# CliqueOfficial/zk-dcap-verifier

Measured on AMD Instinct MI355X. Metric: proofs/hour sgx_dcap_verifier k=19 (create_proof on the GPU: commitments, lookups, grand products, NTTs, evaluate_h, evaluations, SHPLONK, host transcript; witness synthesis excluded), higher is better.
Workload: dtype u32x8 (256-bit Montgomery integers)

## Files before the change

### zk-dcap-verifier_amd/csrc/capi.hip

```cpp
#include <string.h>
#include <new>
#include <system_error>
#include "quotient.h"

namespace zk {
int ntt_set_lds_attr();
int quotient_set_lds_attr();
int domain_lagrange_to_coeff(zk_ctx* ctx, void* d_a, uint32_t k);
int domain_coeff_to_lagrange(zk_ctx* ctx, void* d_a, uint32_t k);
int domain_lagrange_to_coeff_batch(zk_ctx* ctx, void* const* cols, size_t count, uint32_t k);
int domain_coeff_to_extended_batch(zk_ctx* ctx, const void* const* coeffs, void* const* outs, size_t count, uint32_t k, uint32_t ek);
int ntt_dev_batch(zk_ctx* ctx, void* const* h_cols, const void* const* h_srcs, size_t count, uint32_t log_n, const u256& omega, const NttFuse* fuse);
int domain_coeff_to_extended(zk_ctx* ctx, const void* d_coeff, uint32_t k, uint32_t ek, void* d_out);
int domain_extended_to_coeff(zk_ctx* ctx, void* d_a, uint32_t k, uint32_t ek);
int domain_divide_by_vanishing(zk_ctx* ctx, void* d_a, uint32_t k, uint32_t ek);
int fr_vec_op(zk_ctx* ctx, int op, const void* a, const void* b, void* out, size_t n, const u256* scalar);
int permutation_product(zk_ctx* ctx, const void* const* values, const void* const* sigmas, size_t count, uint32_t k, const void* beta, const void* gamma,
                        const void* delta_start, const void* z_init, const void* blinding, uint32_t bf, void* d_z, void* h_last_z);
int lookup_product(zk_ctx* ctx, const void* cin, const void* ctab, const void* pin, const void* ptab, uint32_t k, const void* beta, const void* gamma,
                   const void* blinding, uint32_t bf, void* d_z);
int permutation_product_circuits(zk_ctx* ctx, const void* const* values, const void* const* sigmas, size_t m, size_t n_circuits, uint32_t chunk_len, uint32_t k,
                                 const void* beta, const void* gamma, const void* blinding, uint32_t bf, void* const* d_zs);
int lookup_product_batch(zk_ctx* ctx, const void* const* cols4, size_t count, uint32_t k, const void* beta, const void* gamma, const void* blinding,
                         uint32_t bf, void* const* d_zs);
// ... 181 lines not shown
        t = ctx->tune; timing = ctx->timing;
    }
    std::lock_guard<std::mutex> lk(h->mu);
    h->tune = t;
    h->timing = timing;
    return h;
}
static void release_workspaces(zk_ctx* ctx) {
    zk::DevBuf* bufs[] = {&ctx->ws_scalars, &ctx->ws_sorted, &ctx->ws_mid, &ctx->ws_small, &ctx->ws_sub0, &ctx->ws_sub1, &ctx->ws_cls0,
                          &ctx->ws_cls1, &ctx->ws_tmp, &ctx->ws_ntt, &ctx->ws_ntt_in, &ctx->ws_pts, &ctx->ws_runs, &ctx->ws_quot, &ctx->ws_quot_state};
    for (auto* b : bufs) b->release();
}
void zk_internal_trim_helper(zk_ctx* ctx) {
    if (!ctx) return;
    zk_ctx* h;
    { LOCK; h = ctx->helper; }
    if (!h) return;
    std::lock_guard<std::mutex> lk(h->mu);
    (void)hipSetDevice(h->device);
    (void)hipStreamSynchronize(h->stream);
    release_workspaces(h);
    release_twiddles(h);
}
extern "C" {
void zk_ctx_destroy(zk_ctx* ctx) ZK_ABI_TRY {
    if (!ctx) return;
    zk_ctx* helper;
    { LOCK; helper = ctx->helper; ctx->helper = nullptr; }
    if (helper) zk_ctx_destroy(helper);
    zk_internal_plonk_ctx_destroyed(ctx);
    (void)zk_plonk_trim(ctx);
    {
        LOCK;
        (void)hipSetDevice(ctx->device);
        (void)hipStreamSynchronize(ctx->stream);
        ctx->bases.clear();
        drop_pending_timers(ctx);
        release_twiddles(ctx);
        release_pks(ctx);
        release_mock_sessions(ctx);
        release_programs(ctx);
        release_gtab(ctx);
        release_workspaces(ctx);
        (void)hipStreamDestroy(ctx->stream);
    }
    delete ctx;
} ZK_ABI_CATCH_VOID(ctx)

const char* zk_last_error(zk_ctx* ctx) ZK_ABI_TRY { return ctx ? ctx->err : "null context"; } ZK_ABI_CATCH_VALUE(ctx, "zkmi355: internal error")

static int* tune_slot(zk_ctx* ctx, const char* key) {
    zk::Tune& t = ctx->tune;
    struct { const char* k; int* v; } tab[] = {
        {"msm_c", &t.msm_c}, {"msm_sort_wgs", &t.msm_sort_wgs}, {"msm_sort_threads", &t.msm_sort_threads}, {"msm_sort_batch_wgs", &t.msm_sort_batch_wgs}, {"msm_bsort_threads", &t.msm_bsort_threads}, {"msm_bsort_chunk", &t.msm_bsort_chunk}, {"msm_wide_bins_log", &t.msm_wide_bins_log}, {"msm_part_threads", &t.msm_part_threads}, {"msm_part_pairs", &t.msm_part_pairs}, {"msm_two_level_sort", &t.msm_two_level_sort},
        {"msm_target_threads", &t.msm_target_threads}, {"msm_min_chunk", &t.msm_min_chunk}, {"msm_max_chunk", &t.msm_max_chunk},
        {"msm_max_chunk_wide", &t.msm_max_chunk_wide}, {"msm_merge_fanin", &t.msm_merge_fanin}, {"msm_tree_fanin", &t.msm_tree_fanin}, {"msm_block", &t.msm_block}, {"msm_runs", &t.msm_runs}, {"prover_side_lane", &t.prover_side_lane}, {"prover_lane_priority", &t.prover_lane_priority},
        {"ntt_tile_log", &t.ntt_tile_log}, {"ntt_threads", &t.ntt_threads}, {"ntt_max_radix_log", &t.ntt_max_radix_log}, {"ntt_plan", &t.ntt_plan}, {"ntt_full_twiddle_max_log", &t.ntt_full_twiddle_max_log}, {"ntt_coset_table", &t.ntt_coset_table}, {"ntt_col_major", &t.ntt_col_major},
        {"vec_block", &t.vec_block}, {"quot_threads", &t.quot_threads},
        {"ntt_quarter_input", &t.ntt_quarter_input}, {"ntt_fuse_scale", &t.ntt_fuse_scale}, {"quot_piece_cosets", &t.quot_piece_cosets}, {"quot_factor_horner", &t.quot_factor_horner}, {"quot_degree_split", &t.quot_degree_split}, {"quot_group_factors", &t.quot_group_factors}, {"ntt_ws_limit_mb", &t.ntt_ws_limit_mb}, 
        {"quot_jit", &t.quot_jit}, {"quot_jit_group", &t.quot_jit_group}, {"quot_jit_waves", &t.quot_jit_waves}, {"quot_remat_ops", &t.quot_remat_ops}, {"quot_remat_distance", &t.quot_remat_distance}, {"keygen_wgs", &t.keygen_wgs}, {"mock_edge_wgs", &t.mock_edge_wgs}};
    for (auto& e : tab) if (!strcmp(e.k, key)) return e.v;
    return nullptr;
}
int zk_tune_set(zk_ctx* ctx, const char* key, int value) ZK_ABI_TRY {
    NEED_CTX; LOCK;
    int* s = key ? tune_slot(ctx, key) : nullptr;
    if (!s) return ctx->fail(ZK_ERR_ARG, "zk_tune_set: unknown key '%s'", key ? key : "(null)");
    if (value < 0) return ctx->fail(ZK_ERR_ARG, "zk_tune_set: negative value");
    *s = value;
    return ZK_OK;
} ZK_ABI_CATCH(ctx)
int zk_tune_get(zk_ctx* ctx, const char* key, int* value) ZK_ABI_TRY {
    NEED_CTX; LOCK;
    int* s = key ? tune_slot(ctx, key) : nullptr;
    if (!s || !value) return ctx->fail(ZK_ERR_ARG, "zk_tune_get: unknown key '%s'", key ? key : "(null)");
    *value = *s;
    return ZK_OK;
} ZK_ABI_CATCH(ctx)
int zk_timing_enable(zk_ctx* ctx, int on) ZK_ABI_TRY {
    NEED_CTX;
    zk_ctx* helper;
    { LOCK; helper = ctx->helper; }
    if (helper) (void)zk_timing_enable(helper, on);
    LOCK;
    resolve_pending_timers(ctx);
    if (on) ctx->last_ms.clear();
    ctx->timing = on != 0;
    return ZK_OK;
} ZK_ABI_CATCH(ctx)
double zk_timing_get(zk_ctx* ctx, const char* label) ZK_ABI_TRY {
    if (!ctx || !label) return -1.0;
    zk_ctx* helper;
    { LOCK; helper = ctx->helper; }
    const double side = helper ? zk_timing_get(helper, label) : -1.0;
    LOCK;
    resolve_pending_timers(ctx);
    auto it = ctx->last_ms.find(label);
    if (it == ctx->last_ms.end()) return side;
    return it->second + (side > 0 ? side : 0.0);
} ZK_ABI_CATCH_VALUE(ctx, -1.0)

#define ENTER NEED_CTX; LOCK; ZK_HIP(hipSetDevice(ctx->device))

int zk_dev_alloc(zk_ctx* ctx, size_t bytes, void** dptr) ZK_ABI_TRY { ENTER; if (!dptr) return ctx->fail(ZK_ERR_ARG, "null"); ZK_HIP(hipMalloc(dptr, bytes ? bytes : 32)); return ZK_OK; } ZK_ABI_CATCH(ctx)
int zk_dev_free(zk_ctx* ctx, void* dptr) ZK_ABI_TRY { ENTER; ZK_HIP(hipFree(dptr)); return ZK_OK; } ZK_ABI_CATCH(ctx)
int zk_dev_upload(zk_ctx* ctx, void* dptr, const void* host, size_t bytes) ZK_ABI_TRY {
    ENTER; if ((!dptr || !host) && bytes) return ctx->fail(ZK_ERR_ARG, "zk_dev_upload: null");
// ... 285 lines not shown
```

### zk-dcap-verifier_amd/csrc/ctx.h

```cpp
#pragma once
#include <stdarg.h>
#include <string.h>
#include <stdio.h>
#include <list>
#include <map>
#include <memory>
#include <mutex>
#include <string>
#include <vector>
#include "ec.cuh"
#include "../../include/zkmi355.h"
#include "abi_guard.h"

namespace zk {

struct Tune {
    int msm_c = 0;
    int msm_sort_wgs = 256;
    int msm_sort_threads = 1024;
    int msm_bsort_threads = 1024;
    int msm_bsort_chunk = 8192;
    int msm_part_threads = 1024, msm_part_pairs = 16384;
    int msm_wide_bins_log = 9;
    int msm_two_level_sort = 0;
    int msm_sort_batch_wgs = 2048;
    int msm_target_threads = 1 << 19;
    int msm_min_chunk = 16;
    int msm_max_chunk = 48;
    int msm_max_chunk_wide = 128;
    int msm_merge_fanin = 8;
    int msm_tree_fanin = 2;
    int msm_block = 128;
    int prover_lane_priority = 1;
    int prover_side_lane = 1;
    int msm_runs = 1;
    int ntt_tile_log = 10;
    int ntt_threads = 256;
    int ntt_max_radix_log = 8;
    int ntt_plan = 0;
    int ntt_col_major = 1;
    int ntt_coset_table = 1;
    int ntt_full_twiddle_max_log = 24;
    int ntt_ws_limit_mb = 24576;
    int ntt_fuse_scale = 1;
    int ntt_quarter_input = 1;
    int vec_block = 256;
    int quot_threads = 128;
    int quot_piece_cosets = 1;
    int quot_degree_split = 1;
    int quot_group_factors = 1;
    int quot_factor_horner = 1;
    int quot_remat_ops = 4;
    int quot_remat_distance = 24;
    int quot_jit = 0;
    int quot_jit_waves = 0;
    int keygen_wgs = 2048;
    int mock_edge_wgs = 2048;
    int quot_jit_group = 200;
};

struct DevBuf {
    void* p = nullptr;
    size_t cap = 0;
    hipError_t ensure(size_t bytes) {
        if (bytes <= cap) return hipSuccess;
        if (p) (void)hipFree(p);
        p = nullptr; cap = 0;
        size_t want = bytes + bytes / 8 + 4096;
        hipError_t e = hipMalloc(&p, want);
        if (e == hipSuccess) cap = want;
        return e;
    }
    void release() { if (p) (void)hipFree(p); p = nullptr; cap = 0; }
};

struct DevTmp {
    void* p = nullptr;
    DevTmp() = default;
// ... 81 lines not shown
#define ZK_CHECK_LAUNCH() ZK_HIP(hipGetLastError())

namespace zk {
inline void resolve_pending_timers(zk_ctx* ctx);
struct EvTimer {
    zk_ctx* ctx; const char* label; hipEvent_t a = nullptr, b = nullptr; bool on;
    EvTimer(zk_ctx* c, const char* l) : ctx(c), label(l), on(c->timing) {
        if (on) { (void)hipEventCreate(&a); (void)hipEventCreate(&b); (void)hipEventRecord(a, ctx->stream); }
    }
    void stop() { if (on) (void)hipEventRecord(b, ctx->stream); }
    void resolve() {
        if (!on) return;
        (void)hipEventSynchronize(b);
        float ms = 0; (void)hipEventElapsedTime(&ms, a, b);
        on = false;
        (void)hipEventDestroy(a); (void)hipEventDestroy(b);
        ctx->last_ms[label] += ms; ctx->last_ms[std::string(label) + "#n"] += 1.0;
    }
    void defer() {
        if (!on) return;
        if (ctx->pending_timers.size() >= 4096) resolve_pending_timers(ctx);
        ctx->pending_timers.push_back({label, a, b});
        on = false;
    }
    ~EvTimer() { if (on) { (void)hipEventDestroy(a); (void)hipEventDestroy(b); } }
    EvTimer(const EvTimer&) = delete;
    EvTimer& operator=(const EvTimer&) = delete;
};
inline void resolve_pending_timers(zk_ctx* ctx) {
    std::vector<zk_ctx::PendingTimer> list;
    list.swap(ctx->pending_timers);
    struct Drop { std::vector<zk_ctx::PendingTimer>& l; ~Drop() { for (auto& t : l) { (void)hipEventDestroy(t.a); (void)hipEventDestroy(t.b); } } } drop{list};
    for (auto& t : list) {
        (void)hipEventSynchronize(t.b);
        float ms = 0; (void)hipEventElapsedTime(&ms, t.a, t.b);
        ctx->last_ms[t.label] += ms; ctx->last_ms[std::string(t.label) + "#n"] += 1.0;
    }
}
inline void drop_pending_timers(zk_ctx* ctx) {
    for (auto& t : ctx->pending_timers) { (void)hipEventDestroy(t.a); (void)hipEventDestroy(t.b); }
    ctx->pending_timers.clear();
}

int msm_register(zk_ctx* ctx, const void* pts, size_t n, bool on_device, uint64_t* handle);
int msm_release(zk_ctx* ctx, uint64_t handle);
int msm_share(zk_ctx* dst, const BaseTable& bt, uint64_t* handle);
int msm_enable_runs(zk_ctx* ctx, uint64_t handle);
int msm_run(zk_ctx* ctx, uint64_t handle, const void* scalars, size_t n, bool on_device, void* out, int partial);
int msm_run_batch(zk_ctx* ctx, uint64_t handle, const void* const* scalars, size_t nb, size_t n, bool on_device, void* out, int partial);
int g1_sum_xyzz_host(const void* xyzz, size_t count, void* out_jac);
int g1_fixed_base_mul(zk_ctx* ctx, const void* d_scalars, size_t n, void* d_out_affine);
void release_gtab(zk_ctx* ctx);
int msm_set_lds_attr();
struct NttFuse {
    const void* src = nullptr;
    uint32_t n_valid = 0;
    int pre_zeta = 0;
    int post_scale = 0;
    u256 scale;
    int post_zeta_inv = 0;
    const void* cs_lo = nullptr; const void* cs_hi = nullptr; uint32_t cs_lo_bits = 0, cs_stride = 0, cs_log = 0;
    const void* pre_full = nullptr;
};
int ntt_dev(zk_ctx* ctx, void* d_a, uint32_t log_n, const u256& omega, const NttFuse* fuse);
void release_twiddles(zk_ctx* ctx);
void release_programs(zk_ctx* ctx);
void release_mock_sessions(zk_ctx* ctx);
int quotient_program_share(zk_ctx* ctx, zk_ctx* owner, uint64_t owner_prog, uint64_t* prog);
}
```

### zk-dcap-verifier_amd/csrc/msm.hip

```cpp
#include "ctx.h"
#include <algorithm>
#include <math.h>

namespace zk {

template <class F>
ZK_HD void for_each_digit(u256 s, int c, int W, F&& f) {
    const uint32_t mask = (1u << c) - 1u, half = 1u << (c - 1);
    uint32_t carry = 0;
    for (int j = 0; j < W; j++) {
        uint32_t d = (s.v[0] & mask) + carry;
#pragma unroll
        for (int i = 0; i < 7; i++) s.v[i] = (s.v[i] >> c) | (s.v[i + 1] << (32 - c));
        s.v[7] >>= c;
        if (d > half) {
            carry = 1;
            uint32_t m = (1u << c) - d;
            if (m) f(j, m, true);
        } else {
            carry = 0;
            if (d) f(j, d, false);
        }
    }
}
// ... 28 lines not shown
        if (d > 0x8000u) {
            carry = 1;
            const uint32_t m = 0x10000u - d;
            if (m) f(j, m, true);
        } else {
            carry = 0;
            if (d) f(j, d, false);
        }
    }
}
template <int J = 0, class F>
ZK_HD void for_each_digit16_static(const u256& s, F&& f, uint32_t carry = 0) {
    if constexpr (J < 16) {
        const uint32_t d = ((s.v[J >> 1] >> (16 * (J & 1))) & 0xffffu) + carry;
        uint32_t cy = 0;
        if (d > 0x8000u) {
            cy = 1;
            const uint32_t m = 0x10000u - d;
            if (m) f(WinIdx<J>{}, m, true);
        } else if (d) f(WinIdx<J>{}, d, false);
        for_each_digit16_static<J + 1>(s, f, cy);
    }
}

ZK_HD uint32_t find_segment(const uint32_t* arr, uint32_t B, uint32_t j) {
    uint32_t lo = 0, hi = B;
    while (hi - lo > 1) {
        uint32_t mid = (lo + hi) >> 1;
        if (arr[mid] <= j) lo = mid; else hi = mid;
    }
    return lo;
}

ZK_HD uint32_t ceil_div(uint32_t a, uint32_t b) { return (a + b - 1) / b; }

constexpr int MSM_MAX_LEVELS = 12;
struct MsmPlan {
    uint32_t n, n_table, B, L, M, Mlog, R, nb;
    int c, W;
    const void* const* scalars;
    const void* table;
    const void* const* col_tables;
    uint32_t* small;
    uint32_t small_stride, o_off, o_cursor, o_suboff, o_info, o_tiles, o_fulloff, o_remorder, o_remhist, o_remstart, o_remcursor;
    uint32_t* sorted;
    uint64_t sorted_stride;
    uint32_t low_bits, nbin, pch, bch, o_bintot, o_bincur, o_binbase, o_chunkbase;
    uint32_t* mid_ref;
    uint16_t* mid_low;
    void* sub[2];
    uint64_t sub_stride[2];
    void* cls[2];
    uint32_t lo_bits;
};
ZK_HD uint32_t* plan_small(const MsmPlan& p, uint32_t col) { return p.small + (size_t)col * p.small_stride; }
ZK_HD const uint32_t* plan_suboff(const MsmPlan& p, uint32_t col, uint32_t level) { return plan_small(p, col) + p.o_suboff + (size_t)level * (p.B + 1); }
ZK_HD uint32_t plan_eff_levels(const MsmPlan& p, uint32_t max_s) {
    uint32_t pw = 1, r = 0;
    while (pw < max_s && r < p.R) { pw *= p.M; r++; }
    return r;
}

constexpr uint32_t MSM_MAX_BINS = 2048, MSM_MAX_LOW = 8192;
constexpr int MSM_MAX_C = 22;

__device__ __forceinline__ void block_incscan(uint32_t* v, uint32_t* tmp, uint32_t N) {
    for (uint32_t d = 1; d < N; d <<= 1) {
        for (uint32_t t = threadIdx.x; t < N; t += blockDim.x) tmp[t] = v[t] + (t >= d ? v[t - d] : 0u);
        __syncthreads();
        for (uint32_t t = threadIdx.x; t < N; t += blockDim.x) v[t] = tmp[t];
        __syncthreads();
    }
}

ZK_KERNEL void msm_bin_hist_kernel(MsmPlan p) {
    __shared__ uint32_t lh[MSM_MAX_BINS];
    const uint32_t col = blockIdx.y;
    const void* scalars = p.scalars[col];
    for (uint32_t b = threadIdx.x; b < p.nbin; b += blockDim.x) lh[b] = 0;
    __syncthreads();
    const uint32_t chunk = ceil_div(p.n, gridDim.x);
    const uint32_t lo = blockIdx.x * chunk;
    const uint32_t hi = lo + chunk < p.n ? lo + chunk : p.n;
    for (uint32_t i = lo + threadIdx.x; i < hi; i += blockDim.x) {
        u256 s = Fr::from_mont(load_u256(scalars, i));
        for_each_digit(s, p.c, p.W, [&](int, uint32_t mag, bool) { atomicAdd(&lh[(mag - 1) >> p.low_bits], 1u); });
    }
    __syncthreads();
    uint32_t* tot = plan_small(p, col) + p.o_bintot;
    for (uint32_t b = threadIdx.x; b < p.nbin; b += blockDim.x) {
        uint32_t v = lh[b];
        if (v) atomicAdd(&tot[b], v);
    }
}

ZK_KERNEL void msm_bin_base_kernel(MsmPlan p) {
    __shared__ uint32_t v[MSM_MAX_BINS], w[MSM_MAX_BINS], tmp[MSM_MAX_BINS];
    uint32_t* sm = plan_small(p, blockIdx.x);
    for (uint32_t b = threadIdx.x; b < p.nbin; b += blockDim.x) { const uint32_t t = sm[p.o_bintot + b]; v[b] = t; w[b] = ceil_div(t, p.bch); }
    __syncthreads();
    block_incscan(v, tmp, p.nbin);
    block_incscan(w, tmp, p.nbin);
    for (uint32_t b = threadIdx.x; b < p.nbin; b += blockDim.x) { sm[p.o_binbase + b + 1] = v[b]; sm[p.o_chunkbase + b + 1] = w[b]; }
    if (threadIdx.x == 0) { sm[p.o_binbase] = 0; sm[p.o_chunkbase] = 0; }
}

// ... 85 lines not shown
#pragma unroll
        for (uint32_t u = 0; u < BS_U; u++) { const uint32_t e = e0 + u * blockDim.x; k[u] = e < hi ? mlow[e] : 0xffffffffu; }
#pragma unroll
        for (uint32_t u = 0; u < BS_U; u++) if (k[u] != 0xffffffffu) atomicAdd(&cnt[k[u]], 1u);
    }
    __syncthreads();
    uint32_t* hist = sm + (size_t)bin * nlow;
    for (uint32_t b = threadIdx.x; b < nlow; b += blockDim.x) {
        const uint32_t v = cnt[b];
        if (v) atomicAdd(&hist[b], v);
    }
}
ZK_KERNEL void msm_bsort_place_kernel(MsmPlan p) {
    ZK_DYN_SHARED(uint32_t, cnt);
    const uint32_t col = blockIdx.y, nlow = 1u << p.low_bits;
    uint32_t* sm = plan_small(p, col);
    uint32_t bin, lo, hi;
    if (!bsort_chunk(p, sm, bin, lo, hi)) return;
    for (uint32_t b = threadIdx.x; b < nlow; b += blockDim.x) cnt[b] = 0;
    __syncthreads();
    const uint32_t* __restrict__ mref = p.mid_ref + (size_t)col * p.sorted_stride;
    const uint16_t* __restrict__ mlow = p.mid_low + (size_t)col * p.sorted_stride;
    for (uint32_t e0 = lo + threadIdx.x; e0 < hi; e0 += BS_U * blockDim.x) {
        uint32_t k[BS_U];
#pragma unroll
        for (uint32_t u = 0; u < BS_U; u++) { const uint32_t e = e0 + u * blockDim.x; k[u] = e < hi ? mlow[e] : 0xffffffffu; }
#pragma unroll
        for (uint32_t u = 0; u < BS_U; u++) if (k[u] != 0xffffffffu) atomicAdd(&cnt[k[u]], 1u);
    }
    __syncthreads();
    uint32_t* cursor = sm + p.o_cursor + (size_t)bin * nlow;
    for (uint32_t b0 = threadIdx.x; b0 < nlow; b0 += 4 * blockDim.x) {
        uint32_t v[4], r[4];
#pragma unroll
        for (int u = 0; u < 4; u++) { const uint32_t b = b0 + u * blockDim.x; v[u] = b < nlow ? cnt[b] : 0u; }
#pragma unroll
        for (int u = 0; u < 4; u++) r[u] = v[u] ? atomicAdd(&cursor[b0 + u * blockDim.x], v[u]) : 0u;
#pragma unroll
        for (int u = 0; u < 4; u++) { const uint32_t b = b0 + u * blockDim.x; if (b < nlow) cnt[b] = r[u]; }
    }
    __syncthreads();
    uint32_t* __restrict__ sorted = p.sorted + (size_t)col * p.sorted_stride;
    for (uint32_t e0 = lo + threadIdx.x; e0 < hi; e0 += BS_U * blockDim.x) {
        uint32_t k[BS_U], r[BS_U], d[BS_U];
#pragma unroll
        for (uint32_t u = 0; u < BS_U; u++) { const uint32_t e = e0 + u * blockDim.x; const bool in = e < hi; k[u] = in ? mlow[e] : 0xffffffffu; r[u] = in ? mref[e] : 0u; }
#pragma unroll
        for (uint32_t u = 0; u < BS_U; u++) d[u] = k[u] != 0xffffffffu ? atomicAdd(&cnt[k[u]], 1u) : 0u;
#pragma unroll
        for (uint32_t u = 0; u < BS_U; u++) if (k[u] != 0xffffffffu) sorted[d[u]] = r[u];
    }
}

ZK_KERNEL void msm_hist_kernel(MsmPlan p) {
    ZK_DYN_SHARED(uint32_t, lh);
    const uint32_t B = p.B, col = blockIdx.y;
    const void* scalars = p.scalars[col];
    for (uint32_t b = threadIdx.x; b < B; b += blockDim.x) lh[b] = 0;
    __syncthreads();
    const uint32_t chunk = ceil_div(p.n, gridDim.x);
    const uint32_t lo = blockIdx.x * chunk;
    const uint32_t hi = lo + chunk < p.n ? lo + chunk : p.n;
    const bool wide16 = p.c == 16 && p.W == 16;
    for (uint32_t i = lo + threadIdx.x; i < hi; i += blockDim.x) {
        u256 s = Fr::from_mont(load_u256(scalars, i));
        if (wide16) for_each_digit16(s, [&](int, uint32_t mag, bool) { atomicAdd(&lh[mag - 1], 1u); });
        else for_each_digit(s, p.c, p.W, [&](int, uint32_t mag, bool) { atomicAdd(&lh[mag - 1], 1u); });
    }
    __syncthreads();
    uint32_t* ghist = plan_small(p, col);
    for (uint32_t b = threadIdx.x; b < B; b += blockDim.x) {
        uint32_t v = lh[b];
        if (v) atomicAdd(&ghist[b], v);
    }
}


constexpr uint32_t SC_SPT = 4, SC_WMAX = 32;
ZK_KERNEL void msm_scatter_kernel(MsmPlan p) {
    ZK_DYN_SHARED(uint32_t, lh);
    const uint32_t B = p.B, col = blockIdx.y;
    const void* scalars = p.scalars[col];
    for (uint32_t b = threadIdx.x; b < B; b += blockDim.x) lh[b] = 0;
    const bool wide16 = p.c == 16 && p.W == 16;
    const uint32_t chunk = ceil_div(p.n, gridDim.x);
    const uint32_t lo = blockIdx.x * chunk;
    const uint32_t hi = lo + chunk < p.n ? lo + chunk : p.n;
    u256 sc[SC_SPT];
    uint32_t rk[SC_SPT][SC_WMAX / 2] = {};
#pragma unroll
    for (uint32_t u = 0; u < SC_SPT; u++) {
        const uint32_t i = lo + threadIdx.x + u * blockDim.x;
        if (i < hi) sc[u] = load_u256(scalars, i);
    }
    __syncthreads();
#pragma unroll
    for (uint32_t u = 0; u < SC_SPT; u++) {
        const uint32_t i = lo + threadIdx.x + u * blockDim.x;
        if (i < hi) {
            sc[u] = Fr::from_mont(sc[u]);
            auto count = [&](auto jc, uint32_t mag, bool) {
                constexpr int j = decltype(jc)::value;
                const uint32_t r = atomicAdd(&lh[mag - 1], 1u);
                if (j & 1) rk[u][j / 2] |= r << 16; else rk[u][j / 2] = r;
            };
            if (wide16) for_each_digit16_static(sc[u], count);
            else { u256 t = sc[u]; for_each_digit_static<SC_WMAX>(t, p.c, p.W, count); }
        }
    }
    __syncthreads();
    uint32_t* cursor = plan_small(p, col) + p.o_cursor;
    for (uint32_t b0 = threadIdx.x; b0 < B; b0 += 8 * blockDim.x) {
        uint32_t v[8], r[8];
#pragma unroll
        for (int u = 0; u < 8; u++) { const uint32_t b = b0 + u * blockDim.x; v[u] = b < B ? lh[b] : 0u; }
#pragma unroll
        for (int u = 0; u < 8; u++) r[u] = v[u] ? atomicAdd(&cursor[b0 + u * blockDim.x], v[u]) : 0u;
#pragma unroll
        for (int u = 0; u < 8; u++) { const uint32_t b = b0 + u * blockDim.x; if (b < B) lh[b] = r[u]; }
    }
    __syncthreads();
    uint32_t* sorted = p.sorted + (size_t)col * p.sorted_stride;
#pragma unroll
    for (uint32_t u = 0; u < SC_SPT; u++) {
        const uint32_t i = lo + threadIdx.x + u * blockDim.x;
        if (i < hi) {
            auto place = [&](auto jc, uint32_t mag, bool neg) {
                constexpr int j = decltype(jc)::value;
                const uint32_t r = (j & 1) ? rk[u][j / 2] >> 16 : rk[u][j / 2] & 0xffffu;
                sorted[lh[mag - 1] + r] = (neg ? 0x80000000u : 0u) | ((uint32_t)j * p.n_table + i);
            };
            if (wide16) for_each_digit16_static(sc[u], place);
            else for_each_digit_static<SC_WMAX>(sc[u], p.c, p.W, place);
        }
    }
}

constexpr uint32_t SC_T = 256, SC_E = 4, SC_TILE = SC_T * SC_E, SC_NV = MSM_MAX_LEVELS + 3, REM_CLASSES = 256;
struct ScanVals { uint32_t v[SC_NV]; };
ZK_HD uint32_t rem_class(uint32_t r) { return r < REM_CLASSES ? r : REM_CLASSES - 1; }
ZK_HD void scan_bucket_values(const MsmPlan& p, uint32_t cnt, ScanVals& o, uint32_t& e0) {
    o.v[0] = cnt;
    uint32_t e = ceil_div(cnt, p.L);
    e0 = e;
#pragma unroll
    for (uint32_t r = 0; r <= MSM_MAX_LEVELS + 1; r++) {
        o.v[1 + r] = r <= p.R ? e : (r == p.R + 1 ? cnt / p.L : 0u);
        e = (e + (1u << p.Mlog) - 1) >> p.Mlog;
    }
}
ZK_KERNEL void msm_scan_tiles_kernel(MsmPlan p) {
    __shared__ uint32_t red[SC_T];
    __shared__ uint32_t rh[REM_CLASSES];
    const uint32_t col = blockIdx.y, tile = blockIdx.x, tid = threadIdx.x, B = p.B, NV = p.R + 3;
    uint32_t* sm = plan_small(p, col);
    const uint32_t b0 = tile * SC_TILE + tid * SC_E;
    ScanVals sum;
#pragma unroll
    for (uint32_t v = 0; v < SC_NV; v++) sum.v[v] = 0;
    uint32_t mx = 0;
    for (uint32_t c = tid; c < REM_CLASSES; c += SC_T) rh[c] = 0;
    __syncthreads();
    for (uint32_t e = 0; e < SC_E; e++) {
        const uint32_t b = b0 + e;
        if (b < B) {
            ScanVals x; uint32_t e0;
            const uint32_t cnt = sm[b];
            scan_bucket_values(p, cnt, x, e0);
            mx = e0 > mx ? e0 : mx;
#pragma unroll
            for (uint32_t v = 0; v < SC_NV; v++) sum.v[v] += x.v[v];
            if (cnt % p.L) atomicAdd(&rh[rem_class(cnt % p.L)], 1u);
        }
    }
    __syncthreads();
    for (uint32_t c = tid; c < REM_CLASSES; c += SC_T) if (rh[c]) atomicAdd(&sm[p.o_remhist + c], rh[c]);
    uint32_t* tsum = sm + p.o_tiles + (size_t)tile * SC_NV;
    for (uint32_t v = 0; v <= NV; v++) {
        red[tid] = v < NV ? sum.v[v < SC_NV ? v : 0] : mx;
        __syncthreads();
        for (uint32_t d = SC_T >> 1; d > 0; d >>= 1) {
            if (tid < d) red[tid] = v < NV ? red[tid] + red[tid + d] : (red[tid] > red[tid + d] ? red[tid] : red[tid + d]);
            __syncthreads();
        }
        if (tid == 0) { if (v < NV) tsum[v] = red[0]; else atomicMax(&sm[p.o_info], red[0]); }
        __syncthreads();
// ... 520 lines not shown
    p.o_remorder = p.o_fulloff + B + 1;
    p.o_remhist = p.o_remorder + B;
    p.o_remstart = p.o_remhist + REM_CLASSES;
    p.o_remcursor = p.o_remstart + REM_CLASSES;
    p.o_bintot = p.o_remcursor + REM_CLASSES;
    p.low_bits = c <= 16 ? (uint32_t)std::min(7, c - 1) : (uint32_t)std::max(c - 1 - std::min(std::max(tn.msm_wide_bins_log, 8), 11), 5);
    p.nbin = B >> p.low_bits;
    p.bch = (uint32_t)std::max(64, tn.msm_bsort_chunk);
    p.o_bincur = p.o_bintot + p.nbin;
    p.o_binbase = p.o_bincur + p.nbin;
    p.o_chunkbase = p.o_binbase + p.nbin + 1;
    p.small_stride = p.o_chunkbase + p.nbin + 1;
    const int part_threads = std::min(std::max(tn.msm_part_threads, 64), std::min(1024, tn.msm_sort_threads));
    p.pch = std::min<uint32_t>(std::max<uint32_t>(1, (uint32_t)std::min(std::max(tn.msm_part_pairs, 64), 16384) / (uint32_t)W), PART_SPT * (uint32_t)part_threads);
    if (p.nbin > MSM_MAX_BINS || (1u << p.low_bits) > MSM_MAX_LOW) return ctx->fail(ZK_ERR_LIMIT, "zk_msm: window width c = %d exceeds %d", c, MSM_MAX_C);
    ZK_HIP(ctx->ws_small.ensure((size_t)nb * p.small_stride * 4 + 2 * (size_t)nb * sizeof(void*) + 64));
    p.small = (uint32_t*)ctx->ws_small.p;
    const void** d_ptrs = (const void**)((char*)ctx->ws_small.p + (((size_t)nb * p.small_stride * 4 + 15) & ~(size_t)15));
    p.scalars = d_ptrs;
    p.table = bt.d_table;
    p.col_tables = h_col_tables ? d_ptrs + nb : nullptr;
    p.sorted_stride = (pairs_max + 4 + 15) & ~(uint64_t)15;
    ZK_HIP(ctx->ws_sorted.ensure((size_t)nb * p.sorted_stride * 4));
    p.sorted = (uint32_t*)ctx->ws_sorted.p;
    ZK_HIP(ctx->ws_mid.ensure((size_t)nb * p.sorted_stride * 6 + 64));
    p.mid_ref = (uint32_t*)ctx->ws_mid.p;
    p.mid_low = (uint16_t*)((char*)ctx->ws_mid.p + (size_t)nb * p.sorted_stride * 4);
    p.sub_stride[0] = cap[0];
    p.sub_stride[1] = R >= 1 ? cap[1] : 1;
    ZK_HIP(ctx->ws_sub0.ensure((size_t)nb * p.sub_stride[0] * 128));
    ZK_HIP(ctx->ws_sub1.ensure((size_t)nb * p.sub_stride[1] * 128));
    p.sub[0] = ctx->ws_sub0.p; p.sub[1] = ctx->ws_sub1.p;
    p.lo_bits = (uint32_t)(c - 1 + 1) / 2;
    const uint32_t n_groups = (B >> p.lo_bits) + 1 + (1u << p.lo_bits);
    ZK_HIP(ctx->ws_cls0.ensure((size_t)nb * n_groups * 128));
    ZK_HIP(ctx->ws_cls1.ensure((size_t)nb * c * 128 + 128));
    p.cls[0] = ctx->ws_cls0.p; p.cls[1] = ctx->ws_cls1.p;

    hipStream_t st = ctx->stream;
    ZK_HIP(hipMemsetAsync(p.small, 0, (size_t)nb * p.small_stride * 4, st));
    ZK_HIP(hipMemcpyAsync((void*)d_ptrs, h_scal_ptrs, (size_t)nb * sizeof(void*), hipMemcpyHostToDevice, st));
    if (h_col_tables) ZK_HIP(hipMemcpyAsync((void*)(d_ptrs + nb), h_col_tables, (size_t)nb * sizeof(void*), hipMemcpyHostToDevice, st));
    int wgs = tn.msm_sort_wgs;
    {
        uint64_t per = (uint64_t)tn.msm_sort_threads * 4;
        uint64_t want = (n + per - 1) / per;
        if (want < (uint64_t)wgs) wgs = (int)std::max<uint64_t>(want, 1);
        if (nb > 1) wgs = std::max(1, std::min(wgs, (int)((tn.msm_sort_batch_wgs) / nb) + 1));
    }
    const uint64_t chunk_max = std::min<uint64_t>((uint64_t)SC_SPT * tn.msm_sort_threads, 65536 / (uint64_t)W);
    const uint64_t need = (n + chunk_max - 1) / chunk_max;
    const bool two_level = W > (int)SC_WMAX || c > 16 || tn.msm_two_level_sort != 0;
    const uint32_t bsort_grid = (uint32_t)(pairs_max / p.bch) + p.nbin;
    EvTimer t_sort(ctx, "msm_sort");
    if (two_level) {
        ZK_LAUNCH(msm_bin_hist_kernel, dim3(wgs, nb), tn.msm_sort_threads, 0, st, p);
        ZK_CHECK_LAUNCH();
        ZK_LAUNCH(msm_bin_base_kernel, nb, 256, 0, st, p);
        ZK_CHECK_LAUNCH();
        ZK_LAUNCH(msm_partition_kernel, dim3(ceil_div(p.n, p.pch), nb), part_threads, ((size_t)p.pch * W * 2 + 4 * (size_t)p.nbin) * 4, st, p);
        ZK_CHECK_LAUNCH();
        ZK_LAUNCH(msm_bsort_count_kernel, dim3(bsort_grid, nb), tn.msm_bsort_threads, (size_t)4 << p.low_bits, st, p);
        ZK_CHECK_LAUNCH();
    } else {
        ZK_LAUNCH(msm_hist_kernel, dim3(wgs, nb), tn.msm_sort_threads, (size_t)B * 4, st, p);
        ZK_CHECK_LAUNCH();
    }
    ZK_LAUNCH(msm_scan_tiles_kernel, dim3(scan_tiles, nb), SC_T, 0, st, p);
    ZK_CHECK_LAUNCH();
    ZK_LAUNCH(msm_scan_tilesums_kernel, nb, 64, 0, st, p, scan_tiles);
    ZK_CHECK_LAUNCH();
    ZK_LAUNCH(msm_scan_apply_kernel, dim3(scan_tiles, nb), SC_T, 0, st, p);
    ZK_CHECK_LAUNCH();
    if (two_level) {
        ZK_LAUNCH(msm_bsort_place_kernel, dim3(bsort_grid, nb), tn.msm_bsort_threads, (size_t)4 << p.low_bits, st, p);
        ZK_CHECK_LAUNCH();
    } else {
        ZK_LAUNCH(msm_scatter_kernel, dim3((uint32_t)std::max<uint64_t>(need, (uint64_t)wgs), nb), tn.msm_sort_threads, (size_t)B * 4, st, p);
        ZK_CHECK_LAUNCH();
    }
    t_sort.stop();

    const int blk = tn.msm_block;
    EvTimer t_acc(ctx, "msm_accumulate");
    if (blk > 256) return ctx->fail(ZK_ERR_ARG, "msm_block: at most 256 threads per workgroup");
    {
        const dim3 grid((uint32_t)((cap[0] + blk - 1) / blk), nb);
        ZK_LAUNCH(msm_accumulate_kernel, grid, blk, 0, st, p);
    }
    ZK_CHECK_LAUNCH();
    t_acc.stop();

    EvTimer t_red(ctx, "msm_reduce");
    {
        uint64_t pw = 1;
        for (uint32_t r = 1; r <= R; r++) {
            ZK_LAUNCH(msm_merge_kernel, dim3((uint32_t)((cap[r] + blk - 1) / blk), nb), blk, 0, st, p, r, (uint32_t)std::min<uint64_t>(pw, 0xffffffffull));
            ZK_CHECK_LAUNCH();
            pw *= M;
        }
    }
    if (nb >= 4) { ZK_LAUNCH(msm_rowcol_kernel<16>, dim3((n_groups + 3) / 4, nb), RC_T, 0, st, p); }
    else { ZK_LAUNCH(msm_rowcol_kernel<64>, dim3(n_groups, nb), RC_T, 0, st, p); }
    ZK_CHECK_LAUNCH();
    ZK_LAUNCH(msm_rc_class_kernel, dim3((uint32_t)c, nb), RC_T, 0, st, p);
    ZK_CHECK_LAUNCH();
    t_red.stop();
    std::vector<XYZZ> cls((size_t)nb * c);
    ZK_HIP(hipMemcpyAsync(cls.data(), p.cls[1], (size_t)nb * c * 128, hipMemcpyDeviceToHost, st));
    std::vector<uint32_t> npairs(ctx->timing ? nb : 0);
    for (uint32_t col = 0; col < (uint32_t)npairs.size(); col++)
        ZK_HIP(hipMemcpyAsync(&npairs[col], plan_small(p, col) + p.o_off + B, 4, hipMemcpyDeviceToHost, st));
    ZK_HIP(hipStreamSynchronize(st));
    for (uint32_t v : npairs) ctx->last_ms["msm_pairs"] += (double)v;
    if (ctx->timing) ctx->last_ms["msm_columns"] += (double)nb;
    t_sort.resolve(); t_acc.resolve(); t_red.resolve();
    const int hi_bits = c - (int)p.lo_bits;
    for (uint32_t col = 0; col < nb; col++) {
        const XYZZ* cc = &cls[(size_t)col * c];
        XYZZ h = cc[hi_bits - 1];
        for (int t = hi_bits - 2; t >= 0; t--) { h = xyzz_dbl(h); xyzz_add(h, cc[t]); }
        for (uint32_t t = 0; t < p.lo_bits; t++) h = xyzz_dbl(h);
        XYZZ l = cc[c - 1];
        for (int t = (int)p.lo_bits - 2; t >= 0; t--) { l = xyzz_dbl(l); xyzz_add(l, cc[hi_bits + t]); }
        xyzz_add(h, l);
        out_xyzz[col] = h;
    }
    return ZK_OK;
}

int msm_run_batch(zk_ctx* ctx, uint64_t handle, const void* const* scalars, size_t nb, size_t n, bool on_device, void* out, int partial) {
// ... 141 lines not shown
```

### zk-dcap-verifier_amd/csrc/prover.hip

```cpp
#include <string.h>
#include <algorithm>
#include <atomic>
#include <chrono>
#include <condition_variable>
#include <deque>
#include <functional>
#include <map>
#include <memory>
#include <mutex>
#include <string>
#include <thread>
#include <vector>
#include "field.cuh"
#include "../../include/zkmi355.h"
#include "abi_guard.h"
#include "plonk_shared.h"
#include "transcript.h"

using namespace zk;

zk_ctx* zk_internal_helper_ctx(zk_ctx* ctx);
void zk_internal_trim_helper(zk_ctx* ctx);
int zk_internal_permutation_products(zk_ctx* ctx, const void* const* values, const void* const* sigmas, size_t n_columns, size_t n_circuits, uint32_t chunk_len, uint32_t k,
                                     const void* beta, const void* gamma, const void* blinding, uint32_t blinding_factors, void* const* z_devs);
// ... 748 lines not shown
        for (uint32_t i = 0; i < pk->n_fixed_queries; i++) add(pk->fixed_polys[pk->fixed_queries[2 * i]], rot((int32_t)pk->fixed_queries[2 * i + 1]), once, 0);
        add(random_poly, x, once + 3, 0);
        for (uint32_t j = 0; j < pk->n_perm_columns; j++) add(pk->sigma_polys[j], x, once + 1, 0);
        for (size_t cs = 0; cs < mS; cs++) {
            const uint64_t c = cs / n_sets, s = cs % n_sets;
            add(zs[cs].coef, x, 4 * c + 1, 0);
            add(zs[cs].coef, x_next, 4 * c + 1, 0);
            if (s + 1 < n_sets) add(zs[cs].coef, x_last, 4 * c + 2, n_sets - s);
        }
        for (size_t cl = 0; cl < mL; cl++) {
            const uint64_t c = cl / L, l = cl % L;
            add(lzs[cl].coef, x, 4 * c + 3, 5 * l); add(lzs[cl].coef, x_next, 4 * c + 3, 5 * l + 4);
            add(pin[cl].coef, x, 4 * c + 3, 5 * l + 1); add(pin[cl].coef, x_prev, 4 * c + 3, 5 * l + 3);
            add(ptab[cl].coef, x, 4 * c + 3, 5 * l + 2);
        }
        add(h_poly, x, once + 2, 0);
        std::vector<const void*> polys;
        std::vector<Fe> pts;
        for (const Query& e : q) { polys.push_back(e.poly); pts.push_back(e.point); }
        std::vector<uint64_t> ev(q.size() * 4);
        PK(zk_eval_polynomial_batch_dev(ctx, polys.data(), q.size(), n, packed(pts).data(), ev.data()));
        for (size_t i = 0; i < q.size(); i++) q[i].eval = load32(&ev[4 * i]);
        for (size_t i = 0; i + 1 < q.size(); i++) tr.write_scalar(q[i].eval);
        return ZK_OK;
    }
    int multi_open() {
        std::stable_sort(q.begin(), q.end(), [](const Query& a, const Query& b) { return a.open < b.open; });
        return shplonk_create_proof(ctx, mem, tr, q, n, [this](void* poly) { return commit(pk->srs_g, {poly}); });
    }
    int refused(const char* phase) {
        if (!tr.bad_point) return ZK_OK;
        return pk_fail(ctx, ZK_ERR_ARG, "zk_plonk_create_proof: a commitment of the %s phase is the point at infinity (the committed column is zero on every row): "
                                        "cannot write points at infinity to the transcript", phase);
    }
    int run() {
        PK(validate_and_plan());
        PK(instance_columns());  clk.lap(0);
        PK(advice_columns());    PK(refused("advice"));                  clk.lap(1);
        PK(lookups());           PK(refused("lookup permutation"));      clk.lap(2);
        PK(grand_products());    PK(refused("grand product"));           clk.lap(3);
        PK(random_polynomial()); PK(refused("random polynomial"));       clk.lap(4);
        PK(quotient());          clk.lap(5);
        PK(quotient_pieces());   PK(refused("quotient h(X)"));           clk.lap(6);
        PK(evaluations());       clk.lap(7);
        PK(multi_open());        PK(refused("multi-open"));              clk.lap(8);
        draws.finish();
        *proof_len = tr.out.size();
        if (!proof_out || proof_cap < tr.out.size()) return ZK_ERR_LIMIT;
        memcpy(proof_out, tr.out.data(), tr.out.size());
        return ZK_OK;
    }
};
}

static int create_proof_entry(zk_ctx* ctx, const zk_plonk_pk_desc* pk, uint32_t m, const void* const* advice, int advice_on_device, const void* const* instances,
                              const uint32_t* instance_lens, zk_rng_fn rng, void* rng_user, void* proof_out, size_t proof_cap, size_t* proof_len, const PhaseSpec* ph = nullptr) {
    if (!ctx || !pk) return ZK_ERR_ARG;
    InFlight counted;
    Arena xmem(ctx);
    ShardSignal sig;
    sig.xmem = &xmem;
    int rc;
    try { Proof proof{ctx, pk, m, advice, advice_on_device, instances, instance_lens, rng, rng_user, proof_out, proof_cap, proof_len, sig, ph}; rc = proof.run(); }
    catch (...) { rc = abi_exception(ctx, "zk_plonk_create_proof"); }
    if (rc != ZK_OK && rc != ZK_ERR_COMM && sig.armed && sig.next < sig.sizes.size()) {
        std::string why = zk_last_error(ctx) ? zk_last_error(ctx) : "";
        if (zk_dev_upload(ctx, sig.xsend, POISON, 32) == ZK_OK && zk_dev_sync(ctx) == ZK_OK)
            (void)pk->allgather(pk->allgather_user, sig.xsend, sig.xrecv, sig.sizes[sig.next]);
        pk_fail(ctx, rc, "%s [rank %u of a sharded proof: failure signalled to the other ranks in exchange %zu]", why.c_str(), pk->shard_rank, sig.next);
    }
    return rc;
}

extern "C" int zk_plonk_create_proof(zk_ctx* ctx, const zk_plonk_pk_desc* pk, const void* const* advice, int advice_on_device, const void* const* instances,
                                     const uint32_t* instance_lens, zk_rng_fn rng, void* rng_user, void* proof_out, size_t proof_cap, size_t* proof_len) ZK_ABI_TRY {
    return create_proof_entry(ctx, pk, 1, advice, advice_on_device, instances, instance_lens, rng, rng_user, proof_out, proof_cap, proof_len);
} ZK_ABI_CATCH(ctx)

extern "C" int zk_plonk_create_proof_multi(zk_ctx* ctx, const zk_plonk_pk_desc* pk, uint32_t n_circuits, const void* const* advice, int advice_on_device,
                                           const void* const* instances, const uint32_t* instance_lens, zk_rng_fn rng, void* rng_user,
                                           void* proof_out, size_t proof_cap, size_t* proof_len) ZK_ABI_TRY {
    if (!ctx || !pk) return ZK_ERR_ARG;
    if (!n_circuits) return pk_fail(ctx, ZK_ERR_ARG, "zk_plonk_create_proof_multi: n_circuits = 0");
    return create_proof_entry(ctx, pk, n_circuits, advice, advice_on_device, instances, instance_lens, rng, rng_user, proof_out, proof_cap, proof_len);
} ZK_ABI_CATCH(ctx)

int zk::create_proof_phased(zk_ctx* ctx, const zk_plonk_pk_desc* pk, const PhaseSpec* ph, uint32_t n_circuits, int advice_on_device, const void* const* instances,
                            const uint32_t* instance_lens, zk_rng_fn rng, void* rng_user, void* proof_out, size_t proof_cap, size_t* proof_len) {
    if (!ctx || !pk || !ph) return ZK_ERR_ARG;
    if (!n_circuits) return pk_fail(ctx, ZK_ERR_ARG, "zk_plonk_prove_phased: n_circuits = 0");
    if (pk->n_advice && !ph->advice_out) return ZK_ERR_ARG;
    return create_proof_entry(ctx, pk, n_circuits, ph->advice_out, advice_on_device, instances, instance_lens, rng, rng_user, proof_out, proof_cap, proof_len, ph);
}

extern "C" int zk_plonk_last_challenges(void* out, size_t cap, size_t* n) ZK_ABI_TRY {
    if (!n) return ZK_ERR_ARG;
    const size_t count = g_squeezed.user.size() + g_squeezed.rest.size();
    *n = count;
    if (cap < count * 32 || (count && !out)) return ZK_ERR_LIMIT;
    size_t at = 0;
    for (const std::vector<Fe>* part : {&g_squeezed.user, &g_squeezed.rest})
        for (const Fe& c : *part) { const u256 canon = Fr::from_mont(c); memcpy((char*)out + 32 * at++, canon.v, 32); }
    return ZK_OK;
} ZK_ABI_CATCH(nullptr)

extern "C" int zk_plonk_last_phase_ms(double out[9]) ZK_ABI_TRY {
// ... 21 lines not shown
```

Baseline: 73560.

## Cap MSM sort kernel grids with persistent workgroups looping over work items

The MSM histogram and scatter kernels become grid-stride loops over (column, chunk) work items. When no proofs or many proofs are in flight, the grid is capped at a tunable workgroup count, leaving compute units free for concurrent proofs or side-lane work. Counter zeroing is vectorised with uint4 stores. The cost is fewer resident workgroups for the sort when running alone, plus extra barriers between items.

After: 73910 (median of 4 runs). Within noise of the previous version (+0.5%).

```diff
diff --git a/zk-dcap-verifier_amd/csrc/capi.hip b/zk-dcap-verifier_amd/csrc/capi.hip
--- a/zk-dcap-verifier_amd/csrc/capi.hip
+++ b/zk-dcap-verifier_amd/csrc/capi.hip
@@ -257,7 +257,7 @@
 static int* tune_slot(zk_ctx* ctx, const char* key) {
     zk::Tune& t = ctx->tune;
     struct { const char* k; int* v; } tab[] = {
-        {"msm_c", &t.msm_c}, {"msm_sort_wgs", &t.msm_sort_wgs}, {"msm_sort_threads", &t.msm_sort_threads}, {"msm_sort_batch_wgs", &t.msm_sort_batch_wgs}, {"msm_bsort_threads", &t.msm_bsort_threads}, {"msm_bsort_chunk", &t.msm_bsort_chunk}, {"msm_wide_bins_log", &t.msm_wide_bins_log}, {"msm_part_threads", &t.msm_part_threads}, {"msm_part_pairs", &t.msm_part_pairs}, {"msm_two_level_sort", &t.msm_two_level_sort},
+        {"msm_c", &t.msm_c}, {"msm_sort_wgs", &t.msm_sort_wgs}, {"msm_sort_threads", &t.msm_sort_threads}, {"msm_sort_batch_wgs", &t.msm_sort_batch_wgs}, {"msm_sort_cus", &t.msm_sort_cus}, {"msm_sort_cap_inflight", &t.msm_sort_cap_inflight},{"msm_bsort_threads", &t.msm_bsort_threads}, {"msm_bsort_chunk", &t.msm_bsort_chunk}, {"msm_wide_bins_log", &t.msm_wide_bins_log}, {"msm_part_threads", &t.msm_part_threads}, {"msm_part_pairs", &t.msm_part_pairs}, {"msm_two_level_sort", &t.msm_two_level_sort},
         {"msm_target_threads", &t.msm_target_threads}, {"msm_min_chunk", &t.msm_min_chunk}, {"msm_max_chunk", &t.msm_max_chunk},
         {"msm_max_chunk_wide", &t.msm_max_chunk_wide}, {"msm_merge_fanin", &t.msm_merge_fanin}, {"msm_tree_fanin", &t.msm_tree_fanin}, {"msm_block", &t.msm_block}, {"msm_runs", &t.msm_runs}, {"prover_side_lane", &t.prover_side_lane}, {"prover_lane_priority", &t.prover_lane_priority},
         {"ntt_tile_log", &t.ntt_tile_log}, {"ntt_threads", &t.ntt_threads}, {"ntt_max_radix_log", &t.ntt_max_radix_log}, {"ntt_plan", &t.ntt_plan}, {"ntt_full_twiddle_max_log", &t.ntt_full_twiddle_max_log}, {"ntt_coset_table", &t.ntt_coset_table}, {"ntt_col_major", &t.ntt_col_major},
diff --git a/zk-dcap-verifier_amd/csrc/ctx.h b/zk-dcap-verifier_amd/csrc/ctx.h
--- a/zk-dcap-verifier_amd/csrc/ctx.h
+++ b/zk-dcap-verifier_amd/csrc/ctx.h
@@ -24,6 +24,8 @@
     int msm_wide_bins_log = 9;
     int msm_two_level_sort = 0;
     int msm_sort_batch_wgs = 2048;
+    int msm_sort_cus = 128;
+    int msm_sort_cap_inflight = 3;
     int msm_target_threads = 1 << 19;
     int msm_min_chunk = 16;
     int msm_max_chunk = 48;
@@ -211,6 +213,7 @@
 int g1_fixed_base_mul(zk_ctx* ctx, const void* d_scalars, size_t n, void* d_out_affine);
 void release_gtab(zk_ctx* ctx);
 int msm_set_lds_attr();
+int proofs_in_flight();
 struct NttFuse {
     const void* src = nullptr;
     uint32_t n_valid = 0;
diff --git a/zk-dcap-verifier_amd/csrc/msm.hip b/zk-dcap-verifier_amd/csrc/msm.hip
--- a/zk-dcap-verifier_amd/csrc/msm.hip
+++ b/zk-dcap-verifier_amd/csrc/msm.hip
@@ -104,6 +104,7 @@
     uint64_t sub_stride[2];
     void* cls[2];
     uint32_t lo_bits;
+    uint32_t hist_chunks, scat_chunks;
 };
 ZK_HD uint32_t* plan_small(const MsmPlan& p, uint32_t col) { return p.small + (size_t)col * p.small_stride; }
 ZK_HD const uint32_t* plan_suboff(const MsmPlan& p, uint32_t col, uint32_t level) { return plan_small(p, col) + p.o_suboff + (size_t)level * (p.B + 1); }
@@ -295,26 +296,35 @@
     }
 }
 
+__device__ __forceinline__ void sort_zero_counters(uint32_t* lh, uint32_t B) {
+    uint4* lh4 = reinterpret_cast<uint4*>(lh);
+    for (uint32_t q = threadIdx.x; q < B / 4; q += blockDim.x) lh4[q] = make_uint4(0u, 0u, 0u, 0u);
+    for (uint32_t b = (B & ~3u) + threadIdx.x; b < B; b += blockDim.x) lh[b] = 0;
+}
 ZK_KERNEL void msm_hist_kernel(MsmPlan p) {
     ZK_DYN_SHARED(uint32_t, lh);
-    const uint32_t B = p.B, col = blockIdx.y;
-    const void* scalars = p.scalars[col];
-    for (uint32_t b = threadIdx.x; b < B; b += blockDim.x) lh[b] = 0;
-    __syncthreads();
-    const uint32_t chunk = ceil_div(p.n, gridDim.x);
-    const uint32_t lo = blockIdx.x * chunk;
-    const uint32_t hi = lo + chunk < p.n ? lo + chunk : p.n;
+    const uint32_t B = p.B, chunks = p.hist_chunks, items = chunks * p.nb;
+    const uint32_t chunk = ceil_div(p.n, chunks);
     const bool wide16 = p.c == 16 && p.W == 16;
-    for (uint32_t i = lo + threadIdx.x; i < hi; i += blockDim.x) {
-        u256 s = Fr::from_mont(load_u256(scalars, i));
-        if (wide16) for_each_digit16(s, [&](int, uint32_t mag, bool) { atomicAdd(&lh[mag - 1], 1u); });
-        else for_each_digit(s, p.c, p.W, [&](int, uint32_t mag, bool) { atomicAdd(&lh[mag - 1], 1u); });
-    }
-    __syncthreads();
-    uint32_t* ghist = plan_small(p, col);
-    for (uint32_t b = threadIdx.x; b < B; b += blockDim.x) {
-        uint32_t v = lh[b];
-        if (v) atomicAdd(&ghist[b], v);
+    for (uint32_t item = blockIdx.x; item < items; item += gridDim.x) {
+        const uint32_t col = item / chunks, ck = item % chunks;
+        const void* scalars = p.scalars[col];
+        if (item != blockIdx.x) __syncthreads();
+        sort_zero_counters(lh, B);
+        __syncthreads();
+        const uint32_t lo = ck * chunk;
+        const uint32_t hi = lo + chunk < p.n ? lo + chunk : p.n;
+        for (uint32_t i = lo + threadIdx.x; i < hi; i += blockDim.x) {
+            u256 s = Fr::from_mont(load_u256(scalars, i));
+            if (wide16) for_each_digit16(s, [&](int, uint32_t mag, bool) { atomicAdd(&lh[mag - 1], 1u); });
+            else for_each_digit(s, p.c, p.W, [&](int, uint32_t mag, bool) { atomicAdd(&lh[mag - 1], 1u); });
+        }
+        __syncthreads();
+        uint32_t* ghist = plan_small(p, col);
+        for (uint32_t b = threadIdx.x; b < B; b += blockDim.x) {
+            uint32_t v = lh[b];
+            if (v) atomicAdd(&ghist[b], v);
+        }
     }
 }
 
@@ -322,59 +332,63 @@
 constexpr uint32_t SC_SPT = 4, SC_WMAX = 32;
 ZK_KERNEL void msm_scatter_kernel(MsmPlan p) {
     ZK_DYN_SHARED(uint32_t, lh);
-    const uint32_t B = p.B, col = blockIdx.y;
-    const void* scalars = p.scalars[col];
-    for (uint32_t b = threadIdx.x; b < B; b += blockDim.x) lh[b] = 0;
+    const uint32_t B = p.B, chunks = p.scat_chunks, items = chunks * p.nb;
     const bool wide16 = p.c == 16 && p.W == 16;
-    const uint32_t chunk = ceil_div(p.n, gridDim.x);
-    const uint32_t lo = blockIdx.x * chunk;
-    const uint32_t hi = lo + chunk < p.n ? lo + chunk : p.n;
-    u256 sc[SC_SPT];
-    uint32_t rk[SC_SPT][SC_WMAX / 2] = {};
-#pragma unroll
-    for (uint32_t u = 0; u < SC_SPT; u++) {
-        const uint32_t i = lo + threadIdx.x + u * blockDim.x;
-        if (i < hi) sc[u] = load_u256(scalars, i);
-    }
-    __syncthreads();
-#pragma unroll
-    for (uint32_t u = 0; u < SC_SPT; u++) {
-        const uint32_t i = lo + threadIdx.x + u * blockDim.x;
-        if (i < hi) {
-            sc[u] = Fr::from_mont(sc[u]);
-            auto count = [&](auto jc, uint32_t mag, bool) {
-                constexpr int j = decltype(jc)::value;
-                const uint32_t r = atomicAdd(&lh[mag - 1], 1u);
-                if (j & 1) rk[u][j / 2] |= r << 16; else rk[u][j / 2] = r;
-            };
-            if (wide16) for_each_digit16_static(sc[u], count);
-            else { u256 t = sc[u]; for_each_digit_static<SC_WMAX>(t, p.c, p.W, count); }
-        }
-    }
-    __syncthreads();
-    uint32_t* cursor = plan_small(p, col) + p.o_cursor;
-    for (uint32_t b0 = threadIdx.x; b0 < B; b0 += 8 * blockDim.x) {
-        uint32_t v[8], r[8];
-#pragma unroll
-        for (int u = 0; u < 8; u++) { const uint32_t b = b0 + u * blockDim.x; v[u] = b < B ? lh[b] : 0u; }
-#pragma unroll
-        for (int u = 0; u < 8; u++) r[u] = v[u] ? atomicAdd(&cursor[b0 + u * blockDim.x], v[u]) : 0u;
-#pragma unroll
-        for (int u = 0; u < 8; u++) { const uint32_t b = b0 + u * blockDim.x; if (b < B) lh[b] = r[u]; }
-    }
-    __syncthreads();
-    uint32_t* sorted = p.sorted + (size_t)col * p.sorted_stride;
-#pragma unroll
-    for (uint32_t u = 0; u < SC_SPT; u++) {
-        const uint32_t i = lo + threadIdx.x + u * blockDim.x;
-        if (i < hi) {
-            auto place = [&](auto jc, uint32_t mag, bool neg) {
-                constexpr int j = decltype(jc)::value;
-                const uint32_t r = (j & 1) ? rk[u][j / 2] >> 16 : rk[u][j / 2] & 0xffffu;
-                sorted[lh[mag - 1] + r] = (neg ? 0x80000000u : 0u) | ((uint32_t)j * p.n_table + i);
-            };
-            if (wide16) for_each_digit16_static(sc[u], place);
-            else for_each_digit_static<SC_WMAX>(sc[u], p.c, p.W, place);
+    const uint32_t chunk = ceil_div(p.n, chunks);
+    for (uint32_t item = blockIdx.x; item < items; item += gridDim.x) {
+        const uint32_t col = item / chunks, ck = item % chunks;
+        const void* scalars = p.scalars[col];
+        if (item != blockIdx.x) __syncthreads();
+        sort_zero_counters(lh, B);
+        const uint32_t lo = ck * chunk;
+        const uint32_t hi = lo + chunk < p.n ? lo + chunk : p.n;
+        u256 sc[SC_SPT];
+        uint32_t rk[SC_SPT][SC_WMAX / 2] = {};
+#pragma unroll
+        for (uint32_t u = 0; u < SC_SPT; u++) {
+            const uint32_t i = lo + threadIdx.x + u * blockDim.x;
+            if (i < hi) sc[u] = load_u256(scalars, i);
+        }
+        __syncthreads();
+#pragma unroll
+        for (uint32_t u = 0; u < SC_SPT; u++) {
+            const uint32_t i = lo + threadIdx.x + u * blockDim.x;
+            if (i < hi) {
+                sc[u] = Fr::from_mont(sc[u]);
+                auto count = [&](auto jc, uint32_t mag, bool) {
+                    constexpr int j = decltype(jc)::value;
+                    const uint32_t r = atomicAdd(&lh[mag - 1], 1u);
+                    if (j & 1) rk[u][j / 2] |= r << 16; else rk[u][j / 2] = r;
+                };
+                if (wide16) for_each_digit16_static(sc[u], count);
+                else { u256 t = sc[u]; for_each_digit_static<SC_WMAX>(t, p.c, p.W, count); }
+            }
+        }
+        __syncthreads();
+        uint32_t* cursor = plan_small(p, col) + p.o_cursor;
+        for (uint32_t b0 = threadIdx.x; b0 < B; b0 += 8 * blockDim.x) {
+            uint32_t v[8], r[8];
+#pragma unroll
+            for (int u = 0; u < 8; u++) { const uint32_t b = b0 + u * blockDim.x; v[u] = b < B ? lh[b] : 0u; }
+#pragma unroll
+            for (int u = 0; u < 8; u++) r[u] = v[u] ? atomicAdd(&cursor[b0 + u * blockDim.x], v[u]) : 0u;
+#pragma unroll
+            for (int u = 0; u < 8; u++) { const uint32_t b = b0 + u * blockDim.x; if (b < B) lh[b] = r[u]; }
+        }
+        __syncthreads();
+        uint32_t* sorted = p.sorted + (size_t)col * p.sorted_stride;
+#pragma unroll
+        for (uint32_t u = 0; u < SC_SPT; u++) {
+            const uint32_t i = lo + threadIdx.x + u * blockDim.x;
+            if (i < hi) {
+                auto place = [&](auto jc, uint32_t mag, bool neg) {
+                    constexpr int j = decltype(jc)::value;
+                    const uint32_t r = (j & 1) ? rk[u][j / 2] >> 16 : rk[u][j / 2] & 0xffffu;
+                    sorted[lh[mag - 1] + r] = (neg ? 0x80000000u : 0u) | ((uint32_t)j * p.n_table + i);
+                };
+                if (wide16) for_each_digit16_static(sc[u], place);
+                else for_each_digit_static<SC_WMAX>(sc[u], p.c, p.W, place);
+            }
         }
     }
 }
@@ -1001,6 +1015,14 @@
     const uint64_t need = (n + chunk_max - 1) / chunk_max;
     const bool two_level = W > (int)SC_WMAX || c > 16 || tn.msm_two_level_sort != 0;
     const uint32_t bsort_grid = (uint32_t)(pairs_max / p.bch) + p.nbin;
+    if (tn.msm_sort_cus > 256) return ctx->fail(ZK_ERR_ARG, "msm_sort_cus: 0 (one workgroup per work item) .. 256");
+    p.hist_chunks = (uint32_t)wgs;
+    p.scat_chunks = (uint32_t)std::max<uint64_t>(need, (uint64_t)wgs);
+    const int in_flight = proofs_in_flight();
+    const uint32_t sort_cap = tn.msm_sort_cus > 0 && (in_flight == 0 || in_flight >= tn.msm_sort_cap_inflight) ? ((uint32_t)tn.msm_sort_cus + 7u) & ~7u : 0u;
+    const uint32_t hist_grid = sort_cap ? std::min(sort_cap, p.hist_chunks * nb) : p.hist_chunks * nb;
+    const uint32_t scat_grid = sort_cap ? std::min(sort_cap, p.scat_chunks * nb) : p.scat_chunks * nb;
+    if (ctx->timing && !two_level) { ctx->last_ms["msm_sort_items"] += (double)p.scat_chunks * nb; ctx->last_ms["msm_sort_grid"] += (double)scat_grid; }
     EvTimer t_sort(ctx, "msm_sort");
     if (two_level) {
         ZK_LAUNCH(msm_bin_hist_kernel, dim3(wgs, nb), tn.msm_sort_threads, 0, st, p);
@@ -1012,7 +1034,7 @@
         ZK_LAUNCH(msm_bsort_count_kernel, dim3(bsort_grid, nb), tn.msm_bsort_threads, (size_t)4 << p.low_bits, st, p);
         ZK_CHECK_LAUNCH();
     } else {
-        ZK_LAUNCH(msm_hist_kernel, dim3(wgs, nb), tn.msm_sort_threads, (size_t)B * 4, st, p);
+        ZK_LAUNCH(msm_hist_kernel, hist_grid, tn.msm_sort_threads, (size_t)B * 4, st, p);
         ZK_CHECK_LAUNCH();
     }
     ZK_LAUNCH(msm_scan_tiles_kernel, dim3(scan_tiles, nb), SC_T, 0, st, p);
@@ -1025,7 +1047,7 @@
         ZK_LAUNCH(msm_bsort_place_kernel, dim3(bsort_grid, nb), tn.msm_bsort_threads, (size_t)4 << p.low_bits, st, p);
         ZK_CHECK_LAUNCH();
     } else {
-        ZK_LAUNCH(msm_scatter_kernel, dim3((uint32_t)std::max<uint64_t>(need, (uint64_t)wgs), nb), tn.msm_sort_threads, (size_t)B * 4, st, p);
+        ZK_LAUNCH(msm_scatter_kernel, scat_grid, tn.msm_sort_threads, (size_t)B * 4, st, p);
         ZK_CHECK_LAUNCH();
     }
     t_sort.stop();
diff --git a/zk-dcap-verifier_amd/csrc/prover.hip b/zk-dcap-verifier_amd/csrc/prover.hip
--- a/zk-dcap-verifier_amd/csrc/prover.hip
+++ b/zk-dcap-verifier_amd/csrc/prover.hip
@@ -824,6 +824,7 @@
     }
 };
 }
+namespace zk { int proofs_in_flight() { return g_proofs_in_flight.load(); } }
 
 static int create_proof_entry(zk_ctx* ctx, const zk_plonk_pk_desc* pk, uint32_t m, const void* const* advice, int advice_on_device, const void* const* instances,
                               const uint32_t* instance_lens, zk_rng_fn rng, void* rng_user, void* proof_out, size_t proof_cap, size_t* proof_len, const PhaseSpec* ph = nullptr) {
```
